# CarloSaccardi/GAN-Leaks

Hardware: AMD Instinct MI355X
Metric: attack query-images/sec (10k queries x 100k samples) + AUROC delta vs ref (higher is better)
Workload: dtype split-f16 (hi+lo, f32 accumulate; generator) + i8->i32 exact (distance)

## Files before the change

### gan-leaks_amd/csrc/gl_conv.h

```cpp
#pragma once
#include "gl_common.h"

struct GlGatherConv {
    const float *in;
    unsigned in_bytes;
    int64_t positions;
    int H, W, Cin;
    int up;
    const float *wpack;
    int cols;
    int cols_pad;
    int ntaps;
    uint32_t tap_dy[4], tap_dx[4];
    float *out;
    int Ho, Wo, omul;
    int oy[4], ox[4];
    int planar;
    int64_t ld_planar;
    int out_mode;
    int *sat_flag;
    const float *scale, *shift;
    int cmod;
    int act;
    const float *residual;
// ... 2 lines not shown
    float *tail_out;
    int64_t tail_ld;
    float tail_scale;
    float pixnorm_act;
    const float *rgb_w, *rgb_b;
    float *rgb_out;
    int rgb_n;
    float rgb_inv_act;
    char *tap_V;
    const float *tap_coef;
    int64_t tap_ldv, tap_off;
    int64_t tap_row0;
    int tap_fmt;
    char *tap_pool;
    float tap_scale, tap_eps;
};

static inline bool gl_vrow_blocked(int64_t K1_halves) { return K1_halves * 2 >= (2ll << 20); }
static inline int64_t gl_vrow_capacity(int64_t n, int64_t K1_halves) { return gl_vrow_blocked(K1_halves) ? (n + 255) / 256 * 256 : n; }

#if defined(__HIPCC__)
__device__ __forceinline__ char *gl_vrow_elem(char *V, int64_t ldv, int64_t row, int64_t k)
{
    if (ldv >= 0) return V + row * ldv + k * 2;
    return V + ((row >> 8) * (-ldv) + (k >> 6)) * 32768 + (row & 255) * 128 + (k & 63) * 2;
}

__device__ __forceinline__ float gl_tap_value(float v, float inv, float coef)
{
    float x = v * inv;
    asm volatile("" : "+v"(x));
    float t = x * coef;
    asm volatile("" : "+v"(t));
    return t;
}
#endif
// ... 18 lines not shown
```

### gan-leaks_amd/csrc/gl_conv_h3.hip

```cpp
#include "gl_conv.h"
#include "gl_conv_h3_epi.h"
#include <cstdlib>
#include <type_traits>

namespace {

using gl_h3::v8h;
using gl_h3::v4h;
using gl_h3::v4f;

constexpr int HBK_BYTES = 128;

template <int WC, int WP, int TC = 4, int TP = 4, bool FUSE_TAIL = false, bool UP = false, bool T4 = false>
__global__ void __launch_bounds__(64 * WC * WP, 2) gather_conv_h3_kernel(const GlGatherConv p, int m_tiles, int n_tiles, int phases)
{
#if __HIP_DEVICE_COMPILE__
    constexpr int HTC = 16 * TC * WC, HTP = 16 * TP * WP;
    constexpr int W_BYTES = HTC * HBK_BYTES, X_BYTES = HTP * HBK_BYTES, BUF = W_BYTES + X_BYTES;
    constexpr int NW = WC * WP;
    constexpr int PW = (HTC / 8) / NW, PX = (HTP / 8) / NW;
    static_assert(!T4 || (HTP == 256 && TP == 4 && WP == 4 && PX == 4 && !UP && !FUSE_TAIL), "T4: the 256-position tile with 4 position-waves of 4 fragments");
    extern __shared__ __attribute__((aligned(16))) char smem[];

    const unsigned inner = (unsigned)phases * (unsigned)n_tiles;
    const unsigned id = gl_xcd_remap(blockIdx.x, (unsigned)m_tiles * inner);
    const int mt = (int)(id / inner);
    const int phase = (int)((id % inner) / (unsigned)n_tiles);
    const int nt = (int)(id % (unsigned)n_tiles);
    const int64_t m0 = (int64_t)mt * HTP;
    const int c0 = nt * HTC;

    const int tid0 = threadIdx.x, lane0 = tid0 & 63;
    const int wave = __builtin_amdgcn_readfirstlane(tid0 >> 6);
    const int wc = wave / WP, wp_ = wave % WP;

    const int K = p.ntaps * p.Cin;
    const int nk = K / 32;
    const int HW = p.H * p.W;
    const uint32_t tdy = p.tap_dy[phase], tdx = p.tap_dx[phase];
    const char *wbase = reinterpret_cast<const char *>(p.wpack) + (int64_t)phase * p.cols_pad * K * 4;

    const int rsub = lane0 >> 3, slot = lane0 & 7;
    constexpr int up = UP ? 1 : 0;
    const int Ws = p.W >> up, Hs = p.H >> up;
    constexpr unsigned kOOB = 0xC0000000u;
    const unsigned lead_bytes = (unsigned)(p.W + 1) * (unsigned)p.Cin * 4u;
    const __amdgpu_buffer_rsrc_t x_rsrc =
        __builtin_amdgcn_make_buffer_rsrc(const_cast<char *>(reinterpret_cast<const char *>(p.in)) - (up ? 0 : (int64_t)lead_bytes), 0,
                                          (int)(p.in_bytes + (up ? 0u : 2u * lead_bytes)), 0x00020000);
    const __amdgpu_buffer_rsrc_t w_rsrc = __builtin_amdgcn_make_buffer_rsrc(const_cast<char *>(wbase), 0, (int)((unsigned)p.cols_pad * (unsigned)K * 4u), 0x00020000);
    unsigned x_voff0 = kOOB, x_mask2[(PX + 1) / 2], w_voff0 = 0;
#pragma unroll
    for (int i = 0; i < (PX + 1) / 2; ++i) x_mask2[i] = 0;
    auto x_mask_of = [&](int i) -> unsigned { return (x_mask2[i >> 1] >> ((i & 1) * 16)) & 0xFFFFu; };
    int x_img[UP ? PX : 1], x_yx[UP ? PX : 1];
    {
        const int r = wave * PW * 8 + rsub;
        w_voff0 = ((unsigned)(c0 + r) * (unsigned)K) * 4u + (unsigned)(slot ^ rsub) * 16u;
    }
    const unsigned w_step = 8u * (unsigned)K * 4u, x_step = 8u * (unsigned)p.Cin * 4u;
    auto t4_pos = [](int r) -> int { const int f = r >> 4, wpp = f >> 2, j = f & 3; return (r & 15) * 16 + 4 * j + ((j + wpp) & 3); };
#pragma unroll
    for (int i = 0; i < PX; ++i) {
        const int r = (wave * PX + i) * 8 + rsub;
        const int chunk = slot ^ (r & 7);
        const int64_t pos = m0 + (T4 ? t4_pos(r) : r);
        if constexpr (UP) { x_img[i] = 0; x_yx[i] = 0; }
        if (pos < p.positions) {
            const int64_t img = pos / HW;
            const int rem = (int)(pos - img * HW);
            const int y = rem / p.W, x = rem - y * p.W;
            for (int t = 0; t < p.ntaps; ++t) {
                const int yy = y + (int)((tdy >> (2 * t)) & 3u) - 1, xx = x + (int)((tdx >> (2 * t)) & 3u) - 1;
                if ((yy >= 0) & (yy < p.H) & (xx >= 0) & (xx < p.W)) x_mask2[i >> 1] |= 1u << (t + (i & 1) * 16);
            }
            if (i == 0 || T4) { if (i == 0) x_voff0 = (unsigned)pos * (unsigned)p.Cin * 4u + (unsigned)chunk * 16u; }
            if constexpr (UP) { x_img[i] = (int)(img * Hs * Ws); x_yx[i] = y | (x << 16); }
        }
    }

    auto stage = [&](int kt, char *buf) {
        const int tap = kt % p.ntaps;
        const int cc = kt / p.ntaps;
        const int dy = (int)((tdy >> (2 * tap)) & 3u) - 1;
        const int dx = (int)((tdx >> (2 * tap)) & 3u) - 1;
        const unsigned tapbit = 1u << tap;
#pragma unroll
        for (int i = 0; i < PW; ++i)
            __builtin_amdgcn_raw_ptr_buffer_load_lds(w_rsrc, (gl_lptr)(buf + (wave * PW + i) * 1024), 16, w_voff0, (unsigned)kt * 128u + (unsigned)i * w_step, 0, 0);
        if (!up) {
            const unsigned soff = (unsigned)(((dy + 1) * p.W + (dx + 1)) * p.Cin) * 4u + (unsigned)cc * 128u;
#pragma unroll
            for (int i = 0; i < PX; ++i) {
                const unsigned voff = (x_mask_of(i) & tapbit) ? x_voff0 : kOOB;
                unsigned piece = (unsigned)i * x_step;
                if constexpr (T4) piece = (unsigned)(t4_pos((wave * PX + i) * 8) - t4_pos(wave * PX * 8)) * (unsigned)p.Cin * 4u;
                __builtin_amdgcn_raw_ptr_buffer_load_lds(x_rsrc, (gl_lptr)(buf + W_BYTES + (wave * PX + i) * 1024), 16, voff, soff + piece, 0, 0);
            }
        } else {
            const unsigned soff = (unsigned)cc * 128u;
#pragma unroll
            for (int i = 0; i < PX; ++i) {
                const int r = (wave * PX + i) * 8 + rsub;
                const int yy = (x_yx[UP ? i : 0] & 0xFFFF) + dy, xx = (x_yx[UP ? i : 0] >> 16) + dx;
                const unsigned pix = (unsigned)(x_img[UP ? i : 0] + (yy >> 1) * Ws + (xx >> 1));
                const unsigned voff = (x_mask_of(i) & tapbit) ? pix * (unsigned)p.Cin * 4u + (unsigned)((slot ^ (r & 7)) * 16) : kOOB;
                __builtin_amdgcn_raw_ptr_buffer_load_lds(x_rsrc, (gl_lptr)(buf + W_BYTES + (wave * PX + i) * 1024), 16, voff, soff, 0, 0);
            }
        }
    };

    v4f acc[TC][TP];
#pragma unroll
    for (int i = 0; i < TC; ++i)
#pragma unroll
        for (int j = 0; j < TP; ++j) acc[i][j] = (v4f){0.f, 0.f, 0.f, 0.f};

    const int frow0 = lane0 & 15, fk0 = lane0 >> 4;
    auto compute = [&](const char *cur, int kt) {
        const char *lw = cur + (wc * 16 * TC) * HBK_BYTES;
        const char *lx = cur + W_BYTES + (wp_ * 16 * TP) * HBK_BYTES;
        v8h w_hi[TC], w_lo[TC], x_hi[TP], x_lo[TP];
        unsigned skip = 0;
        if constexpr (T4) {
            const int tap = kt % p.ntaps;
            const int dy = (int)((tdy >> (2 * tap)) & 3u) - 1, dx = (int)((tdx >> (2 * tap)) & 3u) - 1;
#pragma unroll
            for (int j = 0; j < TP; ++j) {
                const int yy = j + dy, xx = ((j + wp_) & 3) + dx;
                skip |= ((yy < 0) | (yy > 3) | (xx < 0) | (xx > 3)) ? 1u << j : 0u;
            }
        }
#pragma unroll
        for (int i = 0; i < TC; ++i) {
            const int r = i * 16 + frow0;
            w_hi[i] = *reinterpret_cast<const v8h *>(lw + r * HBK_BYTES + ((fk0 ^ (r & 7)) << 4));
            w_lo[i] = *reinterpret_cast<const v8h *>(lw + r * HBK_BYTES + (((4 + fk0) ^ (r & 7)) << 4));
        }
#pragma unroll
// ... 12 lines not shown
                    acc[i][j] = __builtin_amdgcn_mfma_f32_16x16x32_f16(w_hi[i], x_lo[j], acc[i][j], 0, 0, 0);
                    acc[i][j] = __builtin_amdgcn_mfma_f32_16x16x32_f16(w_hi[i], x_hi[j], acc[i][j], 0, 0, 0);
                }
            }
        } else {
#pragma unroll
            for (int i = 0; i < TC; ++i)
#pragma unroll
                for (int j = 0; j < TP; ++j) {
                    acc[i][j] = __builtin_amdgcn_mfma_f32_16x16x32_f16(w_lo[i], x_hi[j], acc[i][j], 0, 0, 0);
                    acc[i][j] = __builtin_amdgcn_mfma_f32_16x16x32_f16(w_hi[i], x_lo[j], acc[i][j], 0, 0, 0);
                    acc[i][j] = __builtin_amdgcn_mfma_f32_16x16x32_f16(w_hi[i], x_hi[j], acc[i][j], 0, 0, 0);
                }
        }
    };
    stage(0, smem);
    for (int kt = 0; kt < nk; ++kt) {
        __syncthreads();
        if (kt + 1 < nk) stage(kt + 1, smem + ((kt + 1) & 1) * BUF);
        compute(smem + (kt & 1) * BUF, kt);
    }

    __syncthreads();
    int tid_again = threadIdx.x;
    asm volatile("" : "+v"(tid_again));
    const int tid = tid_again, lane = tid_again & 63, frow = tid_again & 15, fk = (tid_again & 63) >> 4;
    int *orow = reinterpret_cast<int *>(smem);
    if (tid < HTP) {
        const int64_t pos = m0 + (T4 ? t4_pos(tid) : tid);
        int o = -1;
        if (pos < p.positions) {
            const int64_t img = pos / HW;
            const int rem = (int)(pos - img * HW);
            const int y = rem / p.W, x = rem - y * p.W;
            o = (int)((img * p.Ho + (y * p.omul + p.oy[phase])) * p.Wo + (x * p.omul + p.ox[phase]));
        }
        orow[tid] = o;
    }
    __syncthreads();
    int o4[TP];
#pragma unroll
    for (int j = 0; j < TP; ++j) o4[j] = orow[wp_ * 16 * TP + j * 16 + frow];
    const float relu_floor = p.act == 1 ? 0.0f : -__builtin_inff();
    const float neg_slope = p.act == 2 ? 0.2f : 1.0f;
    bool saturated = false;
    if constexpr (FUSE_TAIL) {
        static_assert((WC == 2 || WC == 1) && TC == 4 && TP == 4, "fused tail: waves of 64 channels x 64 positions, 64 or 128 channels in all");
        v8h b_hi[2][TP], b_lo[2][TP];
#pragma unroll
        for (int i = 0; i < TC; ++i) {
            const int ch = wc * 64 + i * 16 + 4 * fk;
            float sc[4], sh[4];
#pragma unroll
            for (int r = 0; r < 4; ++r) { sc[r] = p.scale[ch + r]; sh[r] = p.shift[ch + r]; }
#pragma unroll
            for (int j = 0; j < TP; ++j)
#pragma unroll
                for (int r = 0; r < 4; ++r) {
                    float t = fmaf(acc[i][j][r], sc[r], sh[r]);
                    t = fmaxf(fmaxf(t, t * neg_slope), relu_floor);
                    const float c = fminf(fmaxf(t, -65504.0f), 65504.0f);
                    saturated |= (c != t) && (o4[j] >= 0);
                    const _Float16 h = (_Float16)c;
                    b_hi[i >> 1][j][(i & 1) * 4 + r] = h;
                    b_lo[i >> 1][j][(i & 1) * 4 + r] = (_Float16)(c - (float)h);
                }
        }
        v4f pacc[3][TP];
#pragma unroll
        for (int pt = 0; pt < 3; ++pt)
#pragma unroll
            for (int j = 0; j < TP; ++j) pacc[pt][j] = (v4f){0.f, 0.f, 0.f, 0.f};
        const v8h *tw = reinterpret_cast<const v8h *>(p.tail_w) + (size_t)wc * 3 * 2 * 2 * 64;
#pragma unroll
        for (int pt = 0; pt < 3; ++pt)
#pragma unroll
            for (int s2 = 0; s2 < 2; ++s2) {
                const v8h a_hi = tw[((pt * 2 + s2) * 2 + 0) * 64 + frow * 4 + fk];
                const v8h a_lo = tw[((pt * 2 + s2) * 2 + 1) * 64 + frow * 4 + fk];
#pragma unroll
                for (int j = 0; j < TP; ++j) {
                    pacc[pt][j] = __builtin_amdgcn_mfma_f32_16x16x32_f16(a_lo, b_hi[s2][j], pacc[pt][j], 0, 0, 0);
                    pacc[pt][j] = __builtin_amdgcn_mfma_f32_16x16x32_f16(a_hi, b_lo[s2][j], pacc[pt][j], 0, 0, 0);
                    pacc[pt][j] = __builtin_amdgcn_mfma_f32_16x16x32_f16(a_hi, b_hi[s2][j], pacc[pt][j], 0, 0, 0);
                }
            }
        float *xch = reinterpret_cast<float *>(smem + 4096) + (size_t)wp_ * 3 * TP * 4 * 64;
        if (WC == 2 && wc == 1) {
#pragma unroll
            for (int pt = 0; pt < 3; ++pt)
#pragma unroll
                for (int j = 0; j < TP; ++j)
#pragma unroll
                    for (int r = 0; r < 4; ++r) xch[((pt * TP + j) * 4 + r) * 64 + lane] = pacc[pt][j][r];
        }
        if (WC == 2) __syncthreads();
        if (wc == 0) {
#pragma unroll
            for (int pt = 0; pt < 3; ++pt)
#pragma unroll
                for (int j = 0; j < TP; ++j) {
                    const int o = o4[j];
                    if (o < 0) continue;
#pragma unroll
                    for (int r = 0; r < 4; ++r) {
                        const float v = pacc[pt][j][r] + (WC == 2 ? xch[((pt * TP + j) * 4 + r) * 64 + lane] : 0.0f);
                        p.tail_out[(int64_t)(pt * 16 + 4 * fk + r) * p.tail_ld + o] = v * p.tail_scale;
                    }
                }
        }
    } else {
        saturated |= gl_h3::epilogue<WC, WP, TC, TP>(p, acc, c0, wc, wp_, lane, o4, smem, p.tap_V ? (p.Wo >> 4) : 0);
    }
    if (__any(saturated) && lane == 0) atomicAdd(p.sat_flag, 1);
#endif
}

__global__ void __launch_bounds__(256) split_rows_kernel(const float *__restrict__ in, int64_t n, int d, int dpad, float scale, char *__restrict__ out)
{
    const int64_t i = (int64_t)blockIdx.x * blockDim.x + threadIdx.x;
    if (i >= n * dpad) return;
    const int64_t r = i / dpad;
    const int c = (int)(i - r * dpad);
    const float v = c < d ? fminf(fmaxf(in[r * d + c] * scale, -65504.0f), 65504.0f) : 0.0f;
    const _Float16 hi = (_Float16)v;
    const _Float16 lo = (_Float16)(v - (float)hi);
    char *dst = out + (r * dpad + (c >> 5) * 32) * 4 + (c & 31) * 2;
    *reinterpret_cast<_Float16 *>(dst) = hi;
    *reinterpret_cast<_Float16 *>(dst + 64) = lo;
}

}

template <int WC, int WP, int TC = 4, int TP = 4, bool FUSE_TAIL = false, bool UP = false, bool T4 = false>
static int launch_h3(gl_ctx *ctx, const GlGatherConv &p, int phases)
{
    if constexpr (!UP && !FUSE_TAIL && !T4) {
        if (p.up) return launch_h3<WC, WP, TC, TP, FUSE_TAIL, true>(ctx, p, phases);
    }
    if constexpr (WC == 2 && WP == 4 && TC == 8 && TP == 4 && !UP && !FUSE_TAIL && !T4) {
        const bool plain = !p.up && !p.tail_w && !p.tap_V && !p.rgb_out && p.pixnorm_act == 0.0f && !p.planar;
        if (plain && p.H == 4 && p.W == 4 && gl_tuning_int("GL_H3_T4", 1)) return launch_h3<WC, WP, TC, TP, false, false, true>(ctx, p, phases);
    }
    constexpr int HTC = 16 * TC * WC, HTP = 16 * TP * WP;
    const int64_t m_tiles = gl_ceil_div(p.positions, HTP);
    const int n_tiles = (int)gl_ceil_div(p.cols, HTC);
    GL_REQUIRE(m_tiles * n_tiles * phases < (1ll << 31), "gather_conv_h3: grid too large");
    constexpr int lds = 2 * (HTC + HTP) * HBK_BYTES;
    auto kern = gather_conv_h3_kernel<WC, WP, TC, TP, FUSE_TAIL, UP, T4>;
    GL_ONCE_PER_DEVICE(ctx, \
        GL_HIP(hipFuncSetAttribute(reinterpret_cast<const void *>(kern), hipFuncAttributeMaxDynamicSharedMemorySize, lds)););
    gl_prof_scope prof_(ctx, GL_PROF_GATHER_CONV);
    hipLaunchKernelGGL(kern, dim3((unsigned)(m_tiles * n_tiles * phases)), dim3(64 * WC * WP), lds, ctx->stream, p, (int)m_tiles, n_tiles, phases);
    GL_LAUNCH_CHECK();
    return GL_OK;
}

static int h3_tile_choice(const GlGatherConv &p, int phases)
{
    if (p.tail_w) return p.cols == 128 ? 3 : 4;
    if (p.cols <= 64) return 1;
    if (p.cols % 256 == 0 && gl_ceil_div(p.positions, 256) * (p.cols / 256) * phases >= 256) return 2;
    const int wide128 = gl_tuning_int("GL_H3_TILE128", 1);
    if (wide128 && p.cols <= 128 && gl_ceil_div(p.positions, 512) * phases >= 512) return 5;
// ... 29 lines not shown
    GL_REQUIRE(p.out_mode != 2 || p.cols % 32 == 0, "gather_conv_h3: split output needs cols %% 32 == 0");
    GL_REQUIRE(p.up == 0 || (p.up == 1 && p.H % 2 == 0 && p.W % 2 == 0), "gather_conv_h3: up must be 0 or 1");
    {
        const uint64_t imgs = (uint64_t)(p.positions / ((int64_t)p.H * p.W));
        const uint64_t bytes = imgs * (uint64_t)(p.H >> p.up) * (uint64_t)(p.W >> p.up) * (uint64_t)p.Cin * 4ull;
        GL_REQUIRE(bytes + 2ull * (uint64_t)(p.W + 1) * p.Cin * 4ull < 0xC0000000ull, "gather_conv_h3: input of %llu bytes exceeds 3 GiB; use a smaller pass",
                   (unsigned long long)bytes);
        p.in_bytes = (unsigned)bytes;
    }
    GL_REQUIRE((uint64_t)p.cols_pad * p.ntaps * p.Cin * 4ull < 0xC0000000ull, "gather_conv_h3: packed weights too large");
    if (p.positions == 0) return GL_OK;
    GL_REQUIRE(p.positions < (1ll << 31) && (p.positions / ((int64_t)p.H * p.W)) * p.Ho * p.Wo < (1ll << 31), "gather_conv_h3: too many positions");
    GL_REQUIRE(p.pixnorm_act == 0.0f || (p.out_mode == 2 && !p.tail_w && phases == 1 && p.cols <= gl_conv_h3_tile_channels(p, phases)),
               "gather_conv_h3: the fused PixelNorm needs split output and all %d channels in one tile", p.cols);
    GL_REQUIRE(!p.tap_V || (p.pixnorm_act == 0.0f && p.tap_coef && gl_conv_h3_tap_fusable(p, phases)), "gather_conv_h3: this layer's tap cannot be fused");
    if (p.tail_w)
        GL_REQUIRE(p.up == 0 && (p.cols == 128 || p.cols == 64) && p.cmod == p.cols && p.tail_out && p.tail_ld > 0, "gather_conv_h3: the fused tail needs a 64- or 128-channel layer");
    if (gl_conv_halo_applies(p, phases)) return gl_launch_conv_halo_h3(ctx, p);
    switch (h3_tile_choice(p, phases)) {
    case 3: return launch_h3<2, 2, 4, 4, true>(ctx, p, phases);
    case 4: return launch_h3<1, 4, 4, 4, true>(ctx, p, phases);
    case 1: return launch_h3<1, 4>(ctx, p, phases);
    case 2: return launch_h3<2, 4, 8, 4>(ctx, p, phases);
    case 5: return launch_h3<1, 8, 8, 4>(ctx, p, phases);
    default: return launch_h3<2, 2>(ctx, p, phases);
    }
}

int gl_launch_split_rows(gl_ctx *ctx, const float *in, int64_t n, int d, int dpad, float scale, void *out)
{
// ... 44 lines not shown
```

### gan-leaks_amd/csrc/gl_conv_h3_epi.h

```cpp
#pragma once
#include "gl_conv.h"
#include <type_traits>

namespace gl_h3 {

typedef _Float16 v8h __attribute__((ext_vector_type(8)));
typedef _Float16 v4h __attribute__((ext_vector_type(4)));
typedef float v4f __attribute__((ext_vector_type(4)));

template <int WC, int WP, int TC, int TP>
__device__ __forceinline__ bool epilogue(const GlGatherConv &p, v4f (&acc)[TC][TP], int c0, int wc, int wp_, int lane, const int (&o4)[TP], char *smem,
                                         int pool_dj = 0)
{
    const int frow = lane & 15, fk = lane >> 4;
    const float relu_floor = p.act == 1 ? 0.0f : -__builtin_inff();
    const float neg_slope = p.act == 2 ? 0.2f : 1.0f;
    bool saturated = false;
    constexpr bool kFusable = TC <= 4;
    const bool pixnorm = kFusable && p.pixnorm_act > 0.0f;
    const bool tap = kFusable && p.tap_V != nullptr;
    float pinv[TP];
#pragma unroll
    for (int j = 0; j < TP; ++j) pinv[j] = 1.0f;
    if constexpr (kFusable) if (pixnorm || tap) {
        float tss[TC][TP];
#pragma unroll
        for (int i = 0; i < TC; ++i) {
            const int ch = c0 + wc * 16 * TC + i * 16 + 4 * fk;
            const bool real = ch < p.cols;
            const int chm = ch < p.cmod ? ch : ch % p.cmod;
            float sc[4], sh[4];
#pragma unroll
            for (int r = 0; r < 4; ++r) { sc[r] = real ? p.scale[chm + r] : 0.0f; sh[r] = real ? p.shift[chm + r] : 0.0f; }
#pragma unroll
            for (int j = 0; j < TP; ++j) {
                float s1 = 0.0f;
#pragma unroll
                for (int r = 0; r < 4; ++r) {
                    float t = fmaf(acc[i][j][r], sc[r], sh[r]);
                    t = fmaxf(fmaxf(t, t * neg_slope), relu_floor);
                    const float c = fminf(fmaxf(t, -65504.0f), 65504.0f);
                    saturated |= (c != t) && (o4[j] >= 0);
                    const _Float16 h = (_Float16)c;
                    const float vq = __fadd_rn((float)h, (float)(_Float16)__fsub_rn(c, (float)h));
                    acc[i][j][r] = vq;
                    s1 = fmaf(vq, vq, s1);
                }
                s1 += __shfl_xor(s1, 16, 64);
// ... 33 lines not shown
#pragma unroll
                for (int w = 1; w < NT; w *= 2)
#pragma unroll
                    for (int k = 0; k < NT; k += 2 * w) t[k] = __fadd_rn(t[k], t[k + w]);
                ss[j] = t[0];
            }
        }
        if (tap) {
#pragma unroll
            for (int j = 0; j < TP; ++j) pinv[j] = __fdiv_rn(p.tap_scale, __fadd_rn(__fsqrt_rn(ss[j]), p.tap_eps));
            const int HW = p.Ho * p.Wo, Wp = p.Wo >> 1;
            int img[TP], pin[TP];
#pragma unroll
            for (int j = 0; j < TP; ++j) {
                const int o = o4[j] >= 0 ? o4[j] : 0;
                img[j] = o / HW;
                pin[j] = o - img[j] * HW;
            }
#pragma unroll
            for (int i = 0; i < TC; ++i) {
                const int ch = c0 + wc * 16 * TC + i * 16 + 4 * fk;
                if (ch >= p.cols) continue;
                float cf[4];
#pragma unroll
                for (int r = 0; r < 4; ++r) cf[r] = p.tap_coef[ch + r];
#pragma unroll
                for (int j = 0; j < TP; ++j) {
                    if (o4[j] < 0) continue;
                    v4h oh, ol;
#pragma unroll
                    for (int r = 0; r < 4; ++r) {
// ... 11 lines not shown
                    }
                }
                if (p.tap_pool) {
                    auto pool = [&](auto dj_c) {
                        constexpr int DJ = decltype(dj_c)::value;
#pragma unroll
                        for (int j = 0; j < TP; ++j) {
                            if ((j & DJ) != 0) continue;
                            float m[4];
#pragma unroll
                            for (int r = 0; r < 4; ++r) {
                                m[r] = fmaxf(acc[i][j][r], acc[i][(j ^ DJ) % TP][r]);
                                m[r] = fmaxf(m[r], __shfl_xor(m[r], 1, 64));
                            }
                            if ((frow & 1) != 0 || o4[j] < 0) continue;
                            const int y = pin[j] / p.Wo, x = pin[j] - y * p.Wo;
                            char *dst = p.tap_pool + ((int64_t)img[j] * (HW >> 2) + (y >> 1) * Wp + (x >> 1)) * p.cols * 4 + (ch >> 5) * 128 + (ch & 31) * 2;
                            v4h hi, lo;
#pragma unroll
                            for (int r = 0; r < 4; ++r) {
                                hi[r] = (_Float16)m[r];
                                lo[r] = (_Float16)__fsub_rn(m[r], (float)hi[r]);
                            }
                            *reinterpret_cast<v4h *>(dst) = hi;
                            *reinterpret_cast<v4h *>(dst + 64) = lo;
                        }
                    };
                    if (pool_dj == 1) pool(std::integral_constant<int, 1>());
                    else pool(std::integral_constant<int, 2>());
                }
            }
// ... 61 lines not shown
#pragma unroll
            for (int j = 0; j < TP; ++j) {
                float out4[4];
#pragma unroll
                for (int c = 0; c < 4; ++c) {
                    float sacc = res[j][c];
                    sacc = __fadd_rn(sacc, __shfl_xor(sacc, 16, 64));
                    sacc = __fadd_rn(sacc, __shfl_xor(sacc, 32, 64));
                    out4[c] = c < p.rgb_n ? fmaf(sacc, p.rgb_inv_act, p.rgb_b[c]) : 0.0f;
                }
                if (fk == 0 && o4[j] >= 0) *reinterpret_cast<float4 *>(p.rgb_out + (int64_t)o4[j] * 4) = make_float4(out4[0], out4[1], out4[2], out4[3]);
            }
            return saturated;
        }
    }
#pragma unroll
    for (int i = 0; i < TC; ++i) {
        const int ch = c0 + wc * 16 * TC + i * 16 + 4 * fk;
        if (ch >= p.cols) continue;
        float sc[4] = {0.f, 0.f, 0.f, 0.f}, sh[4] = {0.f, 0.f, 0.f, 0.f};
        if (!pixnorm) {
            const int chm = ch < p.cmod ? ch : ch % p.cmod;
#pragma unroll
            for (int r = 0; r < 4; ++r) { sc[r] = p.scale[chm + r]; sh[r] = p.shift[chm + r]; }
        }
#pragma unroll
        for (int j = 0; j < TP; ++j) {
            const int o = o4[j];
            if (o < 0) continue;
            float v[4];
#pragma unroll
            for (int r = 0; r < 4; ++r) {
                if (pixnorm) {
                    v[r] = __fmul_rn(acc[i][j][r], pinv[j]);
                } else {
                    float t = fmaf(acc[i][j][r], sc[r], sh[r]);
                    v[r] = fmaxf(fmaxf(t, t * neg_slope), relu_floor);
                }
            }
            if (p.out_mode == 2) {
                char *dst = reinterpret_cast<char *>(p.out) + (int64_t)o * p.cols * 4 + (ch >> 5) * 128 + (ch & 31) * 2;
                v4h hi, lo;
#pragma unroll
                for (int r = 0; r < 4; ++r) {
                    const float c = fminf(fmaxf(v[r], -65504.0f), 65504.0f);
                    saturated |= (c != v[r]);
                    hi[r] = (_Float16)c;
                    lo[r] = pixnorm ? (_Float16)fmaf(acc[i][j][r], pinv[j], -(float)hi[r]) : (_Float16)__fsub_rn(c, (float)hi[r]);
                }
                *reinterpret_cast<v4h *>(dst) = hi;
                *reinterpret_cast<v4h *>(dst + 64) = lo;
            } else if (p.planar) {
#pragma unroll
                for (int r = 0; r < 4; ++r) p.out[(int64_t)(ch + r) * p.ld_planar + o] = v[r];
            } else {
                *reinterpret_cast<float4 *>(p.out + (int64_t)o * p.cols + ch) = make_float4(v[0], v[1], v[2], v[3]);
            }
        }
    }
    return saturated;
}

}
```

### gan-leaks_amd/csrc/gl_conv_halo.hip

```cpp
#include "gl_conv.h"
#include "gl_conv_h3_epi.h"
#include <cstdlib>

namespace {

using gl_h3::v4f;
using gl_h3::v8h;

constexpr int BLK = 16;
constexpr int HALO = BLK + 2;
constexpr int HPIX = HALO * HALO;
constexpr int HPIECES = (HPIX + 7) / 8;
constexpr int HBYTES = HPIECES * 1024;
constexpr int halo_bytes(int nw, bool ring) { return ring ? ((HPIECES + nw - 1) / nw) * nw * 1024 : HBYTES; }

template <int WC, bool RING = false>
__global__ void __launch_bounds__(256 * WC, 2) halo_conv_h3_kernel(const GlGatherConv p, int blocks_x, int blocks_per_img, unsigned total_blocks, int diag)
{
#if __HIP_DEVICE_COMPILE__
    constexpr int TC = 4, TP = 4, WP = 4, NW = WC * WP;
    constexpr int HTC = 64 * WC;
    constexpr int W_BYTES = HTC * 128;
    constexpr int NHBUF = WC;
    constexpr int PH = (HPIECES + NW - 1) / NW;
    constexpr int PW = (HTC / 8) / NW;
    constexpr int HB = halo_bytes(NW, RING);
    extern __shared__ __attribute__((aligned(16))) char smem[];
    char *const wbuf = smem + NHBUF * HB;

    const unsigned id = gl_xcd_remap(blockIdx.x, total_blocks);
    const int img = (int)(id / (unsigned)blocks_per_img);
// ... 127 lines not shown
                __builtin_amdgcn_s_barrier();
                __builtin_amdgcn_sched_barrier(0);
                const int s2 = slot == 0 ? 2 : slot - 1;
                if (kt + 2 < nk) stage_w(kt + 2, wbuf + s2 * W_BYTES);
                if (NHBUF == 2 && tap == 0 && more) stage_halo(cc + 1, smem + ((cc + 1) & 1) * HB);
                compute(hb, wbuf + slot * W_BYTES, (tap / 3 - 1) * HALO + (tap % 3 - 1));
                slot = slot == 2 ? 0 : slot + 1;
            }
            if (NHBUF == 1 && more) {
                __builtin_amdgcn_s_barrier();
                stage_halo(cc + 1, smem);
            }
        }
    }

    __syncthreads();
    int o4[TP];
#pragma unroll
    for (int j = 0; j < TP; ++j) o4[j] = (img * p.Ho + y0 + wp_ * 4 + j) * p.Wo + x0 + frow;
    if (diag & 4) {
        float keep = 0.0f;
#pragma unroll
        for (int i = 0; i < TC; ++i)
#pragma unroll
            for (int j = 0; j < TP; ++j) keep += acc[i][j][0] + acc[i][j][1] + acc[i][j][2] + acc[i][j][3];
        if (keep == 123.456f) atomicAdd(p.sat_flag, 1);
        return;
    }
    const bool saturated = gl_h3::epilogue<WC, WP, TC, TP>(p, acc, 0, wc, wp_, lane, o4, smem, 1);
    if (__any(saturated) && lane == 0) atomicAdd(p.sat_flag, 1);
#endif
}

template <int WC, bool RING = false>
int launch_halo(gl_ctx *ctx, const GlGatherConv &p)
{
    const int bx = p.W / BLK, by = p.H / BLK;
    const int64_t imgs = p.positions / ((int64_t)p.H * p.W);
    const int64_t total = imgs * bx * by;
    GL_REQUIRE(total < (1ll << 31), "halo_conv_h3: grid too large");
    constexpr int lds = WC * halo_bytes(4 * WC, RING) + (RING ? 3 : 2) * 64 * WC * 128;
    auto kern = halo_conv_h3_kernel<WC, RING>;
    GL_ONCE_PER_DEVICE(ctx, \
        GL_HIP(hipFuncSetAttribute(reinterpret_cast<const void *>(kern), hipFuncAttributeMaxDynamicSharedMemorySize, lds)););
    gl_prof_scope prof_(ctx, GL_PROF_GATHER_CONV);
    hipLaunchKernelGGL(kern, dim3((unsigned)total), dim3(256 * WC), lds, ctx->stream, p, bx, bx * by, (unsigned)total, gl_tuning_int("GL_HALO_DIAG", 0));
    GL_LAUNCH_CHECK();
    return GL_OK;
}

}

bool gl_conv_halo_applies(const GlGatherConv &p, int phases)
{
    const int enabled = gl_tuning_int("GL_H3_HALO", 1);
    if (!enabled || phases != 1 || p.ntaps != 9 || p.tail_w || p.cols > 128 || p.Cin % 32 != 0) return false;
    uint32_t dy = 0, dx = 0;
// ... 15 lines not shown
```

Measured before the change: 53180.

## Add lean gather-conv path with fast division, precomputed tap masks and hoisted epilogue constants

Adds a LEAN template path, on by default, to the gather conv and halo kernels. It replaces 64-bit integer division with host-computed magic-number fast division and builds per-position tap validity masks from precomputed border bitmasks. It also splits K-loop staging into prepare and issue steps with scalar offsets, and hoists scale/shift loads, tail weights and output addresses out of the epilogue loops. The goal is less integer ALU and address work and fewer scattered loads per tile, at the cost of extra live registers that could reduce occupancy, plus 32-bit position arithmetic that limits problem size.

```diff
diff --git a/gan-leaks_amd/csrc/gl_conv.h b/gan-leaks_amd/csrc/gl_conv.h
--- a/gan-leaks_amd/csrc/gl_conv.h
+++ b/gan-leaks_amd/csrc/gl_conv.h
@@ -40,12 +40,26 @@
     int tap_fmt;
     char *tap_pool;
     float tap_scale, tap_eps;
+    unsigned hw_magic, w_magic, cmod_magic;
+    int hw_shift, w_shift, cmod_shift;
+    uint32_t tap_tb[4], tap_lr[4];
 };
+
+static inline void gl_fastdiv_init(unsigned d, unsigned &magic, int &shift)
+{
+    int s = 0;
+    while (s < 31 && (1u << s) < d) ++s;
+    if ((1u << s) == d) { magic = 0; shift = s; return; }
+    magic = (unsigned)((1ull << (31 + s)) / d + 1ull);
+    shift = s - 1;
+}
 
 static inline bool gl_vrow_blocked(int64_t K1_halves) { return K1_halves * 2 >= (2ll << 20); }
 static inline int64_t gl_vrow_capacity(int64_t n, int64_t K1_halves) { return gl_vrow_blocked(K1_halves) ? (n + 255) / 256 * 256 : n; }
 
 #if defined(__HIPCC__)
+__device__ __forceinline__ unsigned gl_fastdiv(unsigned n, unsigned magic, int shift) { return (magic ? __umulhi(n, magic) : n) >> shift; }
+
 __device__ __forceinline__ char *gl_vrow_elem(char *V, int64_t ldv, int64_t row, int64_t k)
 {
     if (ldv >= 0) return V + row * ldv + k * 2;
diff --git a/gan-leaks_amd/csrc/gl_conv_h3.hip b/gan-leaks_amd/csrc/gl_conv_h3.hip
--- a/gan-leaks_amd/csrc/gl_conv_h3.hip
+++ b/gan-leaks_amd/csrc/gl_conv_h3.hip
@@ -11,7 +11,7 @@
 
 constexpr int HBK_BYTES = 128;
 
-template <int WC, int WP, int TC = 4, int TP = 4, bool FUSE_TAIL = false, bool UP = false, bool T4 = false>
+template <int WC, int WP, int TC = 4, int TP = 4, bool FUSE_TAIL = false, bool UP = false, bool T4 = false, bool LEAN = true>
 __global__ void __launch_bounds__(64 * WC * WP, 2) gather_conv_h3_kernel(const GlGatherConv p, int m_tiles, int n_tiles, int phases)
 {
 #if __HIP_DEVICE_COMPILE__
@@ -28,6 +28,7 @@
     const int phase = (int)((id % inner) / (unsigned)n_tiles);
     const int nt = (int)(id % (unsigned)n_tiles);
     const int64_t m0 = (int64_t)mt * HTP;
+    const unsigned m0u = (unsigned)mt * (unsigned)HTP, npos = (unsigned)p.positions;
     const int c0 = nt * HTC;
 
     const int tid0 = threadIdx.x, lane0 = tid0 & 63;
@@ -40,6 +41,12 @@
     const uint32_t tdy = p.tap_dy[phase], tdx = p.tap_dx[phase];
     const char *wbase = reinterpret_cast<const char *>(p.wpack) + (int64_t)phase * p.cols_pad * K * 4;
 
+    const unsigned all_taps = (1u << p.ntaps) - 1u;
+    const unsigned b_tb = p.tap_tb[phase], b_lr = p.tap_lr[phase];
+    const unsigned b_top = b_tb & 0xFFFFu, b_bot = b_tb >> 16, b_left = b_lr & 0xFFFFu, b_right = b_lr >> 16;
+    auto border_mask = [&](int y, int x) -> unsigned {
+        return all_taps & ~((y == 0 ? b_top : 0u) | (y == p.H - 1 ? b_bot : 0u) | (x == 0 ? b_left : 0u) | (x == p.W - 1 ? b_right : 0u));
+    };
     const int rsub = lane0 >> 3, slot = lane0 & 7;
     constexpr int up = UP ? 1 : 0;
     const int Ws = p.W >> up, Hs = p.H >> up;
@@ -64,8 +71,20 @@
     for (int i = 0; i < PX; ++i) {
         const int r = (wave * PX + i) * 8 + rsub;
         const int chunk = slot ^ (r & 7);
+        if constexpr (UP) { x_img[i] = 0; x_yx[i] = 0; }
+        if constexpr (LEAN) {
+            const unsigned pos = m0u + (unsigned)(T4 ? t4_pos(r) : r);
+            if (pos < npos) {
+                const unsigned img = gl_fastdiv(pos, p.hw_magic, p.hw_shift);
+                const unsigned rem = pos - img * (unsigned)HW;
+                const int y = (int)gl_fastdiv(rem, p.w_magic, p.w_shift), x = (int)rem - y * p.W;
+                x_mask2[i >> 1] |= border_mask(y, x) << ((i & 1) * 16);
+                if (i == 0) x_voff0 = pos * (unsigned)p.Cin * 4u + (unsigned)chunk * 16u;
+                if constexpr (UP) { x_img[i] = (int)(img * (unsigned)(Hs * Ws)); x_yx[i] = y | (x << 16); }
+            }
+            continue;
+        }
         const int64_t pos = m0 + (T4 ? t4_pos(r) : r);
-        if constexpr (UP) { x_img[i] = 0; x_yx[i] = 0; }
         if (pos < p.positions) {
             const int64_t img = pos / HW;
             const int rem = (int)(pos - img * HW);
@@ -79,7 +98,7 @@
         }
     }
 
-    auto stage = [&](int kt, char *buf) {
+    [[maybe_unused]] auto stage = [&](int kt, char *buf) {
         const int tap = kt % p.ntaps;
         const int cc = kt / p.ntaps;
         const int dy = (int)((tdy >> (2 * tap)) & 3u) - 1;
@@ -110,6 +129,71 @@
         }
     };
 
+    const unsigned cin4 = (unsigned)p.Cin * 4u, wcin4 = (unsigned)p.W * cin4;
+    int nx_tap = 0;
+    unsigned nx_cc = 0, nx_bit = 1u, nx_voff[PX], nx_xs[PX], nx_ws[PW], nx_lds = 0;
+    unsigned st_mask2 = 0, cp_mask[(TP + 1) / 2];
+    if constexpr (T4 && LEAN) {
+#pragma unroll
+        for (int h = 0; h < 2; ++h) {
+            const int f = ((wave * PX) >> 1) + h, wpp = f >> 2, j = f & 3;
+            st_mask2 |= border_mask(j, (j + wpp) & 3) << (16 * h);
+        }
+#pragma unroll
+        for (int j = 0; j < (TP + 1) / 2; ++j) cp_mask[j] = 0;
+#pragma unroll
+        for (int j = 0; j < TP; ++j) cp_mask[j >> 1] |= border_mask(j, (j + wp_) & 3) << (16 * (j & 1));
+    }
+    auto prepare = [&](int kt) {
+        nx_lds = (unsigned)(kt & 1) * (unsigned)BUF;
+#pragma unroll
+        for (int i = 0; i < PW; ++i) nx_ws[i] = (unsigned)kt * 128u + (unsigned)i * w_step;
+        unsigned nx_soff;
+        const int dy1 = (int)((tdy >> (2 * nx_tap)) & 3u), dx1 = (int)((tdx >> (2 * nx_tap)) & 3u);
+        nx_bit = 1u << nx_tap;
+        if constexpr (!UP) {
+            nx_soff = (unsigned)dy1 * wcin4 + (unsigned)dx1 * cin4 + nx_cc;
+#pragma unroll
+            for (int i = 0; i < PX; ++i) nx_voff[i] = (x_mask_of(i) & nx_bit) ? x_voff0 : kOOB;
+        } else {
+            nx_soff = nx_cc;
+#pragma unroll
+            for (int i = 0; i < PX; ++i) {
+                const int r = (wave * PX + i) * 8 + rsub;
+                const int yy = (x_yx[UP ? i : 0] & 0xFFFF) + dy1 - 1, xx = (x_yx[UP ? i : 0] >> 16) + dx1 - 1;
+                const unsigned pix = (unsigned)(x_img[UP ? i : 0] + (yy >> 1) * Ws + (xx >> 1));
+                nx_voff[i] = (x_mask_of(i) & nx_bit) ? pix * cin4 + (unsigned)((slot ^ (r & 7)) * 16) : kOOB;
+            }
+        }
+#pragma unroll
+        for (int i = 0; i < PX; ++i) {
+            unsigned piece = UP ? 0u : (unsigned)i * x_step;
+            if constexpr (T4) piece = (unsigned)(t4_pos((wave * PX + i) * 8) - t4_pos(wave * PX * 8)) * cin4;
+            nx_xs[i] = nx_soff + piece;
+        }
+        asm volatile("" : "+s"(nx_lds));
+#pragma unroll
+        for (int i = 0; i < PW; ++i) asm volatile("" : "+s"(nx_ws[i]));
+#pragma unroll
+        for (int i = 0; i < PX; ++i) asm volatile("" : "+s"(nx_xs[i]), "+v"(nx_voff[i]));
+    };
+    auto advance = [&]() {
+        if (++nx_tap == p.ntaps) { nx_tap = 0; nx_cc += 128u; }
+    };
+    auto issue = [&]() {
+        char *buf = smem + nx_lds;
+#pragma unroll
+        for (int i = 0; i < PW; ++i)
+            __builtin_amdgcn_raw_ptr_buffer_load_lds(w_rsrc, (gl_lptr)(buf + (wave * PW + i) * 1024), 16, w_voff0, nx_ws[i], 0, 0);
+#pragma unroll
+        for (int i = 0; i < PX; ++i) {
+            if constexpr (T4) {
+                if (!((st_mask2 >> (16 * (i >> 1))) & nx_bit)) continue;
+            }
+            __builtin_amdgcn_raw_ptr_buffer_load_lds(x_rsrc, (gl_lptr)(buf + W_BYTES + (wave * PX + i) * 1024), 16, nx_voff[i], nx_xs[i], 0, 0);
+        }
+    };
+
     v4f acc[TC][TP];
 #pragma unroll
     for (int i = 0; i < TC; ++i)
@@ -117,12 +201,15 @@
         for (int j = 0; j < TP; ++j) acc[i][j] = (v4f){0.f, 0.f, 0.f, 0.f};
 
     const int frow0 = lane0 & 15, fk0 = lane0 >> 4;
-    auto compute = [&](const char *cur, int kt) {
+    auto compute = [&](const char *cur, int kt, unsigned tapbit) {
         const char *lw = cur + (wc * 16 * TC) * HBK_BYTES;
         const char *lx = cur + W_BYTES + (wp_ * 16 * TP) * HBK_BYTES;
         v8h w_hi[TC], w_lo[TC], x_hi[TP], x_lo[TP];
         unsigned skip = 0;
-        if constexpr (T4) {
+        if constexpr (T4 && LEAN) {
+#pragma unroll
+            for (int j = 0; j < TP; ++j) skip |= ((cp_mask[j >> 1] >> (16 * (j & 1))) & tapbit) ? 0u : 1u << j;
+        } else if constexpr (T4) {
             const int tap = kt % p.ntaps;
             const int dy = (int)((tdy >> (2 * tap)) & 3u) - 1, dx = (int)((tdx >> (2 * tap)) & 3u) - 1;
 #pragma unroll
@@ -165,19 +252,45 @@
                 }
         }
     };
-    stage(0, smem);
-    for (int kt = 0; kt < nk; ++kt) {
-        __syncthreads();
-        if (kt + 1 < nk) stage(kt + 1, smem + ((kt + 1) & 1) * BUF);
-        compute(smem + (kt & 1) * BUF, kt);
+    if constexpr (LEAN) {
+        prepare(0);
+        issue();
+        for (int kt = 0; kt < nk; ++kt) {
+            const unsigned tapbit = nx_bit;
+            advance();
+            prepare(kt + 1);
+            __syncthreads();
+            if (kt + 1 < nk) issue();
+            compute(smem + (kt & 1) * BUF, kt, tapbit);
+        }
+    } else {
+        stage(0, smem);
+        for (int kt = 0; kt < nk; ++kt) {
+            __syncthreads();
+            if (kt + 1 < nk) stage(kt + 1, smem + ((kt + 1) & 1) * BUF);
+            compute(smem + (kt & 1) * BUF, kt, 0u);
+        }
     }
 
     __syncthreads();
     int tid_again = threadIdx.x;
     asm volatile("" : "+v"(tid_again));
     const int tid = tid_again, lane = tid_again & 63, frow = tid_again & 15, fk = (tid_again & 63) >> 4;
+    gl_h3::EpiConsts<TC> ec;
+    if constexpr (LEAN && (FUSE_TAIL || TC > 4)) gl_h3::load_epi_consts<TC>(p, (FUSE_TAIL ? 0 : c0) + wc * 16 * TC + 4 * fk, ec);
     int *orow = reinterpret_cast<int *>(smem);
-    if (tid < HTP) {
+    if (LEAN && tid < HTP) {
+        const unsigned pos = m0u + (unsigned)(T4 ? t4_pos(tid) : tid);
+        int o = -1;
+        if (pos < npos) {
+            const unsigned img = gl_fastdiv(pos, p.hw_magic, p.hw_shift);
+            const unsigned rem = pos - img * (unsigned)HW;
+            const int y = (int)gl_fastdiv(rem, p.w_magic, p.w_shift), x = (int)rem - y * p.W;
+            o = ((int)img * p.Ho + (y * p.omul + p.oy[phase])) * p.Wo + (x * p.omul + p.ox[phase]);
+        }
+        orow[tid] = o;
+    }
+    if (!LEAN && tid < HTP) {
         const int64_t pos = m0 + (T4 ? t4_pos(tid) : tid);
         int o = -1;
         if (pos < p.positions) {
@@ -198,12 +311,26 @@
     if constexpr (FUSE_TAIL) {
         static_assert((WC == 2 || WC == 1) && TC == 4 && TP == 4, "fused tail: waves of 64 channels x 64 positions, 64 or 128 channels in all");
         v8h b_hi[2][TP], b_lo[2][TP];
+        const v8h *tw = reinterpret_cast<const v8h *>(p.tail_w) + (size_t)wc * 3 * 2 * 2 * 64;
+        v8h ta_hi[3][2], ta_lo[3][2];
+        if constexpr (LEAN) {
+#pragma unroll
+            for (int pt = 0; pt < 3; ++pt)
+#pragma unroll
+                for (int s2 = 0; s2 < 2; ++s2) {
+                    ta_hi[pt][s2] = tw[((pt * 2 + s2) * 2 + 0) * 64 + frow * 4 + fk];
+                    ta_lo[pt][s2] = tw[((pt * 2 + s2) * 2 + 1) * 64 + frow * 4 + fk];
+                }
+        }
 #pragma unroll
         for (int i = 0; i < TC; ++i) {
             const int ch = wc * 64 + i * 16 + 4 * fk;
             float sc[4], sh[4];
 #pragma unroll
-            for (int r = 0; r < 4; ++r) { sc[r] = p.scale[ch + r]; sh[r] = p.shift[ch + r]; }
+            for (int r = 0; r < 4; ++r) {
+                if constexpr (LEAN) { sc[r] = ec.sc[i][r]; sh[r] = ec.sh[i][r]; }
+                else { sc[r] = p.scale[ch + r]; sh[r] = p.shift[ch + r]; }
+            }
 #pragma unroll
             for (int j = 0; j < TP; ++j)
 #pragma unroll
@@ -222,13 +349,12 @@
         for (int pt = 0; pt < 3; ++pt)
 #pragma unroll
             for (int j = 0; j < TP; ++j) pacc[pt][j] = (v4f){0.f, 0.f, 0.f, 0.f};
-        const v8h *tw = reinterpret_cast<const v8h *>(p.tail_w) + (size_t)wc * 3 * 2 * 2 * 64;
 #pragma unroll
         for (int pt = 0; pt < 3; ++pt)
 #pragma unroll
             for (int s2 = 0; s2 < 2; ++s2) {
-                const v8h a_hi = tw[((pt * 2 + s2) * 2 + 0) * 64 + frow * 4 + fk];
-                const v8h a_lo = tw[((pt * 2 + s2) * 2 + 1) * 64 + frow * 4 + fk];
+                const v8h a_hi = LEAN ? ta_hi[pt][s2] : tw[((pt * 2 + s2) * 2 + 0) * 64 + frow * 4 + fk];
+                const v8h a_lo = LEAN ? ta_lo[pt][s2] : tw[((pt * 2 + s2) * 2 + 1) * 64 + frow * 4 + fk];
 #pragma unroll
                 for (int j = 0; j < TP; ++j) {
                     pacc[pt][j] = __builtin_amdgcn_mfma_f32_16x16x32_f16(a_lo, b_hi[s2][j], pacc[pt][j], 0, 0, 0);
@@ -247,6 +373,9 @@
         }
         if (WC == 2) __syncthreads();
         if (wc == 0) {
+            float *trow[4];
+#pragma unroll
+            for (int r = 0; r < 4; ++r) trow[r] = p.tail_out + (int64_t)(4 * fk + r) * p.tail_ld;
 #pragma unroll
             for (int pt = 0; pt < 3; ++pt)
 #pragma unroll
@@ -256,12 +385,13 @@
 #pragma unroll
                     for (int r = 0; r < 4; ++r) {
                         const float v = pacc[pt][j][r] + (WC == 2 ? xch[((pt * TP + j) * 4 + r) * 64 + lane] : 0.0f);
-                        p.tail_out[(int64_t)(pt * 16 + 4 * fk + r) * p.tail_ld + o] = v * p.tail_scale;
+                        if constexpr (LEAN) trow[r][(int64_t)(pt * 16) * p.tail_ld + o] = v * p.tail_scale;
+                        else p.tail_out[(int64_t)(pt * 16 + 4 * fk + r) * p.tail_ld + o] = v * p.tail_scale;
                     }
                 }
         }
     } else {
-        saturated |= gl_h3::epilogue<WC, WP, TC, TP>(p, acc, c0, wc, wp_, lane, o4, smem, p.tap_V ? (p.Wo >> 4) : 0);
+        saturated |= gl_h3::epilogue<WC, WP, TC, TP, LEAN>(p, acc, c0, wc, wp_, lane, o4, smem, ec, p.tap_V ? (p.Wo >> 4) : 0);
     }
     if (__any(saturated) && lane == 0) atomicAdd(p.sat_flag, 1);
 #endif
@@ -283,22 +413,27 @@
 
 }
 
-template <int WC, int WP, int TC = 4, int TP = 4, bool FUSE_TAIL = false, bool UP = false, bool T4 = false>
+template <int WC, int WP, int TC = 4, int TP = 4, bool FUSE_TAIL = false, bool UP = false, bool T4 = false, bool LEAN = true>
 static int launch_h3(gl_ctx *ctx, const GlGatherConv &p, int phases)
 {
+#ifdef GL_TUNING
+    if constexpr (LEAN) {
+        if (!gl_tuning_int("GL_H3_LEAN", 1)) return launch_h3<WC, WP, TC, TP, FUSE_TAIL, UP, T4, false>(ctx, p, phases);
+    }
+#endif
     if constexpr (!UP && !FUSE_TAIL && !T4) {
-        if (p.up) return launch_h3<WC, WP, TC, TP, FUSE_TAIL, true>(ctx, p, phases);
+        if (p.up) return launch_h3<WC, WP, TC, TP, FUSE_TAIL, true, false, LEAN>(ctx, p, phases);
     }
     if constexpr (WC == 2 && WP == 4 && TC == 8 && TP == 4 && !UP && !FUSE_TAIL && !T4) {
         const bool plain = !p.up && !p.tail_w && !p.tap_V && !p.rgb_out && p.pixnorm_act == 0.0f && !p.planar;
-        if (plain && p.H == 4 && p.W == 4 && gl_tuning_int("GL_H3_T4", 1)) return launch_h3<WC, WP, TC, TP, false, false, true>(ctx, p, phases);
+        if (plain && p.H == 4 && p.W == 4 && gl_tuning_int("GL_H3_T4", 1)) return launch_h3<WC, WP, TC, TP, false, false, true, LEAN>(ctx, p, phases);
     }
     constexpr int HTC = 16 * TC * WC, HTP = 16 * TP * WP;
     const int64_t m_tiles = gl_ceil_div(p.positions, HTP);
     const int n_tiles = (int)gl_ceil_div(p.cols, HTC);
     GL_REQUIRE(m_tiles * n_tiles * phases < (1ll << 31), "gather_conv_h3: grid too large");
     constexpr int lds = 2 * (HTC + HTP) * HBK_BYTES;
-    auto kern = gather_conv_h3_kernel<WC, WP, TC, TP, FUSE_TAIL, UP, T4>;
+    auto kern = gather_conv_h3_kernel<WC, WP, TC, TP, FUSE_TAIL, UP, T4, LEAN>;
     GL_ONCE_PER_DEVICE(ctx, \
         GL_HIP(hipFuncSetAttribute(reinterpret_cast<const void *>(kern), hipFuncAttributeMaxDynamicSharedMemorySize, lds)););
     gl_prof_scope prof_(ctx, GL_PROF_GATHER_CONV);
@@ -358,6 +493,20 @@
     GL_REQUIRE(p.pixnorm_act == 0.0f || (p.out_mode == 2 && !p.tail_w && phases == 1 && p.cols <= gl_conv_h3_tile_channels(p, phases)),
                "gather_conv_h3: the fused PixelNorm needs split output and all %d channels in one tile", p.cols);
     GL_REQUIRE(!p.tap_V || (p.pixnorm_act == 0.0f && p.tap_coef && gl_conv_h3_tap_fusable(p, phases)), "gather_conv_h3: this layer's tap cannot be fused");
+    gl_fastdiv_init((unsigned)(p.H * p.W), p.hw_magic, p.hw_shift);
+    gl_fastdiv_init((unsigned)p.W, p.w_magic, p.w_shift);
+    gl_fastdiv_init((unsigned)p.cmod, p.cmod_magic, p.cmod_shift);
+    for (int ph = 0; ph < phases; ++ph) {
+        p.tap_tb[ph] = p.tap_lr[ph] = 0;
+        for (int t = 0; t < p.ntaps; ++t) {
+            const unsigned dy1 = (p.tap_dy[ph] >> (2 * t)) & 3u, dx1 = (p.tap_dx[ph] >> (2 * t)) & 3u;
+            GL_REQUIRE(dy1 <= 2 && dx1 <= 2, "gather_conv_h3: tap %d of phase %d is not an offset in {-1, 0, 1}", t, ph);
+            if (dy1 == 0) p.tap_tb[ph] |= 1u << t;
+            if (dy1 == 2) p.tap_tb[ph] |= 1u << (16 + t);
+            if (dx1 == 0) p.tap_lr[ph] |= 1u << t;
+            if (dx1 == 2) p.tap_lr[ph] |= 1u << (16 + t);
+        }
+    }
     if (p.tail_w)
         GL_REQUIRE(p.up == 0 && (p.cols == 128 || p.cols == 64) && p.cmod == p.cols && p.tail_out && p.tail_ld > 0, "gather_conv_h3: the fused tail needs a 64- or 128-channel layer");
     if (gl_conv_halo_applies(p, phases)) return gl_launch_conv_halo_h3(ctx, p);
diff --git a/gan-leaks_amd/csrc/gl_conv_h3_epi.h b/gan-leaks_amd/csrc/gl_conv_h3_epi.h
--- a/gan-leaks_amd/csrc/gl_conv_h3_epi.h
+++ b/gan-leaks_amd/csrc/gl_conv_h3_epi.h
@@ -8,9 +8,27 @@
 typedef _Float16 v4h __attribute__((ext_vector_type(4)));
 typedef float v4f __attribute__((ext_vector_type(4)));
 
-template <int WC, int WP, int TC, int TP>
+typedef float v4f_a4 __attribute__((ext_vector_type(4), aligned(4)));
+template <int TC>
+struct EpiConsts {
+    v4f sc[TC], sh[TC];
+};
+__device__ __forceinline__ void load_epi_const_tile(const GlGatherConv &p, int ch, v4f &sc, v4f &sh)
+{
+    const unsigned chm = (unsigned)ch - gl_fastdiv((unsigned)ch, p.cmod_magic, p.cmod_shift) * (unsigned)p.cmod;
+    sc = *reinterpret_cast<const v4f_a4 *>(p.scale + chm);
+    sh = *reinterpret_cast<const v4f_a4 *>(p.shift + chm);
+}
+template <int TC>
+__device__ __forceinline__ void load_epi_consts(const GlGatherConv &p, int ch0, EpiConsts<TC> &ec)
+{
+#pragma unroll
+    for (int i = 0; i < TC; ++i) load_epi_const_tile(p, ch0 + i * 16, ec.sc[i], ec.sh[i]);
+}
+
+template <int WC, int WP, int TC, int TP, bool LEAN = true>
 __device__ __forceinline__ bool epilogue(const GlGatherConv &p, v4f (&acc)[TC][TP], int c0, int wc, int wp_, int lane, const int (&o4)[TP], char *smem,
-                                         int pool_dj = 0)
+                                         const EpiConsts<TC> &ec, int pool_dj = 0)
 {
     const int frow = lane & 15, fk = lane >> 4;
     const float relu_floor = p.act == 1 ? 0.0f : -__builtin_inff();
@@ -28,10 +46,15 @@
         for (int i = 0; i < TC; ++i) {
             const int ch = c0 + wc * 16 * TC + i * 16 + 4 * fk;
             const bool real = ch < p.cols;
-            const int chm = ch < p.cmod ? ch : ch % p.cmod;
+            const int chm = LEAN ? 0 : ch < p.cmod ? ch : ch % p.cmod;
+            v4f sc4, sh4;
+            if constexpr (LEAN) load_epi_const_tile(p, ch, sc4, sh4);
             float sc[4], sh[4];
 #pragma unroll
-            for (int r = 0; r < 4; ++r) { sc[r] = real ? p.scale[chm + r] : 0.0f; sh[r] = real ? p.shift[chm + r] : 0.0f; }
+            for (int r = 0; r < 4; ++r) {
+                if constexpr (LEAN) { sc[r] = real ? sc4[r] : 0.0f; sh[r] = real ? sh4[r] : 0.0f; }
+                else { sc[r] = real ? p.scale[chm + r] : 0.0f; sh[r] = real ? p.shift[chm + r] : 0.0f; }
+            }
 #pragma unroll
             for (int j = 0; j < TP; ++j) {
                 float s1 = 0.0f;
@@ -95,7 +118,7 @@
 #pragma unroll
             for (int j = 0; j < TP; ++j) {
                 const int o = o4[j] >= 0 ? o4[j] : 0;
-                img[j] = o / HW;
+                img[j] = LEAN ? (int)gl_fastdiv((unsigned)o, p.hw_magic, p.hw_shift) : o / HW;
                 pin[j] = o - img[j] * HW;
             }
 #pragma unroll
@@ -137,7 +160,7 @@
                                 m[r] = fmaxf(m[r], __shfl_xor(m[r], 1, 64));
                             }
                             if ((frow & 1) != 0 || o4[j] < 0) continue;
-                            const int y = pin[j] / p.Wo, x = pin[j] - y * p.Wo;
+                            const int y = LEAN ? (int)gl_fastdiv((unsigned)pin[j], p.w_magic, p.w_shift) : pin[j] / p.Wo, x = pin[j] - y * p.Wo;
                             char *dst = p.tap_pool + ((int64_t)img[j] * (HW >> 2) + (y >> 1) * Wp + (x >> 1)) * p.cols * 4 + (ch >> 5) * 128 + (ch & 31) * 2;
                             v4h hi, lo;
 #pragma unroll
@@ -229,12 +252,32 @@
             return saturated;
         }
     }
+    const int ch0 = c0 + wc * 16 * TC + 4 * fk;
+    EpiConsts<TC> ecl;
+    if constexpr (LEAN && kFusable) {
+        if (!pixnorm) load_epi_consts<TC>(p, ch0, ecl);
+    }
+    const EpiConsts<TC> &ecs = kFusable ? ecl : ec;
+    char *oaddr[TP];
+    float *ocol[4];
+    if constexpr (LEAN) {
+        const int lane_off = p.out_mode == 2 ? (ch0 >> 5) * 128 + (ch0 & 31) * 2 : ch0 * 4;
+#pragma unroll
+        for (int j = 0; j < TP; ++j) oaddr[j] = reinterpret_cast<char *>(p.out) + (int64_t)o4[j] * p.cols * 4 + lane_off;
+#pragma unroll
+        for (int r = 0; r < 4; ++r) ocol[r] = p.out + (int64_t)(ch0 + r) * p.ld_planar;
+    }
 #pragma unroll
     for (int i = 0; i < TC; ++i) {
         const int ch = c0 + wc * 16 * TC + i * 16 + 4 * fk;
         if (ch >= p.cols) continue;
         float sc[4] = {0.f, 0.f, 0.f, 0.f}, sh[4] = {0.f, 0.f, 0.f, 0.f};
-        if (!pixnorm) {
+        if constexpr (LEAN) {
+            if (!pixnorm) {
+#pragma unroll
+                for (int r = 0; r < 4; ++r) { sc[r] = ecs.sc[i][r]; sh[r] = ecs.sh[i][r]; }
+            }
+        } else if (!pixnorm) {
             const int chm = ch < p.cmod ? ch : ch % p.cmod;
 #pragma unroll
             for (int r = 0; r < 4; ++r) { sc[r] = p.scale[chm + r]; sh[r] = p.shift[chm + r]; }
@@ -254,7 +297,7 @@
                 }
             }
             if (p.out_mode == 2) {
-                char *dst = reinterpret_cast<char *>(p.out) + (int64_t)o * p.cols * 4 + (ch >> 5) * 128 + (ch & 31) * 2;
+                char *dst = LEAN ? oaddr[j] + ((i >> 1) * 128 + (i & 1) * 32) : reinterpret_cast<char *>(p.out) + (int64_t)o * p.cols * 4 + (ch >> 5) * 128 + (ch & 31) * 2;
                 v4h hi, lo;
 #pragma unroll
                 for (int r = 0; r < 4; ++r) {
@@ -267,9 +310,13 @@
                 *reinterpret_cast<v4h *>(dst + 64) = lo;
             } else if (p.planar) {
 #pragma unroll
-                for (int r = 0; r < 4; ++r) p.out[(int64_t)(ch + r) * p.ld_planar + o] = v[r];
+                for (int r = 0; r < 4; ++r) {
+                    if constexpr (LEAN) ocol[r][(int64_t)(i * 16) * p.ld_planar + o] = v[r];
+                    else p.out[(int64_t)(ch + r) * p.ld_planar + o] = v[r];
+                }
             } else {
-                *reinterpret_cast<float4 *>(p.out + (int64_t)o * p.cols + ch) = make_float4(v[0], v[1], v[2], v[3]);
+                float *dst = LEAN ? reinterpret_cast<float *>(oaddr[j] + i * 64) : p.out + (int64_t)o * p.cols + ch;
+                *reinterpret_cast<float4 *>(dst) = make_float4(v[0], v[1], v[2], v[3]);
             }
         }
     }
diff --git a/gan-leaks_amd/csrc/gl_conv_halo.hip b/gan-leaks_amd/csrc/gl_conv_halo.hip
--- a/gan-leaks_amd/csrc/gl_conv_halo.hip
+++ b/gan-leaks_amd/csrc/gl_conv_halo.hip
@@ -14,7 +14,7 @@
 constexpr int HBYTES = HPIECES * 1024;
 constexpr int halo_bytes(int nw, bool ring) { return ring ? ((HPIECES + nw - 1) / nw) * nw * 1024 : HBYTES; }
 
-template <int WC, bool RING = false>
+template <int WC, bool RING = false, bool LEAN = true>
 __global__ void __launch_bounds__(256 * WC, 2) halo_conv_h3_kernel(const GlGatherConv p, int blocks_x, int blocks_per_img, unsigned total_blocks, int diag)
 {
 #if __HIP_DEVICE_COMPILE__
@@ -172,6 +172,7 @@
         }
     }
 
+    gl_h3::EpiConsts<TC> ec;
     __syncthreads();
     int o4[TP];
 #pragma unroll
@@ -185,20 +186,25 @@
         if (keep == 123.456f) atomicAdd(p.sat_flag, 1);
         return;
     }
-    const bool saturated = gl_h3::epilogue<WC, WP, TC, TP>(p, acc, 0, wc, wp_, lane, o4, smem, 1);
+    const bool saturated = gl_h3::epilogue<WC, WP, TC, TP, LEAN>(p, acc, 0, wc, wp_, lane, o4, smem, ec, 1);
     if (__any(saturated) && lane == 0) atomicAdd(p.sat_flag, 1);
 #endif
 }
 
-template <int WC, bool RING = false>
+template <int WC, bool RING = false, bool LEAN = true>
 int launch_halo(gl_ctx *ctx, const GlGatherConv &p)
 {
+#ifdef GL_TUNING
+    if constexpr (LEAN) {
+        if (!gl_tuning_int("GL_H3_LEAN", 1)) return launch_halo<WC, RING, false>(ctx, p);
+    }
+#endif
     const int bx = p.W / BLK, by = p.H / BLK;
     const int64_t imgs = p.positions / ((int64_t)p.H * p.W);
     const int64_t total = imgs * bx * by;
     GL_REQUIRE(total < (1ll << 31), "halo_conv_h3: grid too large");
     constexpr int lds = WC * halo_bytes(4 * WC, RING) + (RING ? 3 : 2) * 64 * WC * 128;
-    auto kern = halo_conv_h3_kernel<WC, RING>;
+    auto kern = halo_conv_h3_kernel<WC, RING, LEAN>;
     GL_ONCE_PER_DEVICE(ctx, \
         GL_HIP(hipFuncSetAttribute(reinterpret_cast<const void *>(kern), hipFuncAttributeMaxDynamicSharedMemorySize, lds)););
     gl_prof_scope prof_(ctx, GL_PROF_GATHER_CONV);
```

Result: no change. 53140 (median of 2 runs) (-0.1%).
